# whxhcj/multimodal-S2UT

Hardware: AMD Instinct MI355X
Metric: audio-frames/sec/node, mm_s2ut_transformer fp16, max-tokens 40000, 1/2/4/8 GPUs (higher is better)
Workload: dtype fp16; 1 GPU; mm_s2ut_transformer base (ViT-768 image feats, multimodal_attention+gate); model=mm_s2ut_transformer, parallelism=dp1, front_end=GPU fbank+CMVN in step

## Files before the change

### multimodal-s2ut_amd/csrc/gemm.hip

```cpp
#include <stdlib.h>

#include <algorithm>
#include <mutex>

#include "gemm_common.h"

namespace {

#include "gemm_skinny.h"

template <bool KC>
MMS_DEV void load_tile(const h16* __restrict__ X, long ld, int rows_total, int kdim,
                       int row0, int k0, int kend, s16x8 (&r)[4]) {
  const int t = threadIdx.x;
#pragma unroll
  for (int i = 0; i < 4; ++i) {
    const int id = t + i * NT;
    s16x8 v = {0, 0, 0, 0, 0, 0, 0, 0};
    if (KC) {
      const int row = id >> 3, c = id & 7;
      const int gr = row0 + row, gk = k0 + c * 8;
      if (gr < rows_total) {
        const h16* src = X + (long)gr * ld + gk;
        if (gk + 8 <= kend) {
          v = *reinterpret_cast<const s16x8*>(src);
        } else {
#pragma unroll
          for (int e = 0; e < 8; ++e)
            if (gk + e < kend) v[e] = reinterpret_cast<const short*>(src)[e];
        }
      }
    } else {
      const int kr = id >> 4, c = id & 15;
      const int gk = k0 + kr, gr = row0 + c * 8;
      if (gk < kend) {
        const h16* src = X + (long)gk * ld + gr;
        if (gr + 8 <= rows_total) {
          v = *reinterpret_cast<const s16x8*>(src);
        } else {
#pragma unroll
          for (int e = 0; e < 8; ++e)
            if (gr + e < rows_total) v[e] = reinterpret_cast<const short*>(src)[e];
        }
      }
    }
    r[i] = v;
  }
  (void)kdim;
}

template <bool KC>
MMS_DEV void store_tile(char* lds, const s16x8 (&r)[4]) {
  const int t = threadIdx.x;
#pragma unroll
  for (int i = 0; i < 4; ++i) {
    const int id = t + i * NT;
    int off;
    if (KC) {
      const int row = id >> 3, c = id & 7;
      off = row * 128 + ((c ^ (row & 7)) << 4);
    } else {
      const int kr = id >> 4, c = id & 15;
      off = kr * 256 + ((c ^ swz_mn(kr)) << 4);
    }
    *reinterpret_cast<s16x8*>(lds + off) = r[i];
  }
}

template <bool A_KC, bool B_KC, int EPI>
__global__ void __launch_bounds__(NT, 2) gemm_kernel(GemmP P, int tiles_m, int tiles_n, int total) {
  const unsigned long long t_start = P.stamps ? stamp_now() : 0ull;
  if (P.thresh) P.seed = mms_step_seed(P.seed);
  __shared__ __attribute__((aligned(16))) char smem[4 * TILE_BYTES];
  int z, tm, tn;
  tile_coords(blockIdx.x, tiles_m, tiles_n, total, z, tm, tn, P.group_m);
  const int zb = z / P.splitk, zs = z % P.splitk;
  const int z1 = zb / P.bdiv, z2 = zb % P.bdiv;
  const h16* A = P.A + z1 * P.sA1 + z2 * P.sA2;
  const h16* B = P.B + z1 * P.sB1 + z2 * P.sB2;
  const int kbeg = zs * P.kchunk;
  const int kend = min(P.K, kbeg + P.kchunk);
  const int bm = tm * BM, bn = tn * BN;
  const int lane = threadIdx.x & 63, wid = threadIdx.x >> 6;
  const int wm = wid >> 1, wn = wid & 1;

#define SA(s) (smem + (2 * (s)) * TILE_BYTES)
#define SB(s) (smem + (2 * (s) + 1) * TILE_BYTES)

  f32x4 acc[4][4];
#pragma unroll
  for (int i = 0; i < 4; ++i)
#pragma unroll
    for (int j = 0; j < 4; ++j) acc[i][j] = f32x4{0.f, 0.f, 0.f, 0.f};

  s16x8 ra[4], rb[4];
  const int nk = (kend - kbeg + BK - 1) / BK;
  if (nk > 0) {
    load_tile<A_KC>(A, P.lda, P.M, P.K, bm, kbeg, kend, ra);
    load_tile<B_KC>(B, P.ldb, P.N, P.K, bn, kbeg, kend, rb);
    store_tile<A_KC>(SA(0), ra);
    store_tile<B_KC>(SB(0), rb);
  }
  __syncthreads();
  for (int kt = 0; kt < nk; ++kt) {
    const int cur = kt & 1;
    const bool more = kt + 1 < nk;
    if (more) {
      const int k0 = kbeg + (kt + 1) * BK;
      load_tile<A_KC>(A, P.lda, P.M, P.K, bm, k0, kend, ra);
      load_tile<B_KC>(B, P.ldb, P.N, P.K, bn, k0, kend, rb);
    }
#pragma unroll
    for (int kk = 0; kk < 2; ++kk) {
      h16x8 fa[4], fb[4];
#pragma unroll
      for (int i = 0; i < 4; ++i) fa[i] = read_frag<A_KC>(SA(cur), wm * 64 + i * 16, kk, lane);
#pragma unroll
      for (int j = 0; j < 4; ++j) fb[j] = read_frag<B_KC>(SB(cur), wn * 64 + j * 16, kk, lane);
#pragma unroll
      for (int i = 0; i < 4; ++i)
#pragma unroll
        for (int j = 0; j < 4; ++j)
          acc[i][j] = __builtin_amdgcn_mfma_f32_16x16x32_f16(fb[j], fa[i], acc[i][j], 0, 0, 0);
    }
    if (more) {
      store_tile<A_KC>(SA(cur ^ 1), ra);
      store_tile<B_KC>(SB(cur ^ 1), rb);
    }
    __syncthreads();
  }
#undef SA
#undef SB

  char* Cz;
  if (EPI == MMS_EPI_F32)
    Cz = reinterpret_cast<char*>(P.C) + (z1 * P.sC1 + z2 * P.sC2 + zs * P.sCsplit) * 4;
  else
    Cz = reinterpret_cast<char*>(P.C) + (z1 * P.sC1 + z2 * P.sC2) * 2;
  const h16* auxz = P.aux ? P.aux + z1 * P.sX1 + z2 * P.sX2 : nullptr;
  staged_epilogue<EPI>(P, smem, acc, bm, bn, wm, wn, wid, lane, Cz, auxz);
  stamp_end(P.stamps, t_start);
}




template <bool A_KC, bool B_KC, int EPI, int STAGES, bool RS, bool PRI>
MMS_DEV void dma_gemm_tile(const GemmP& P, char* smem, int z, int tm, int tn) {
  const int zb = z / P.splitk, zs = z % P.splitk;
  const int z1 = zb / P.bdiv, z2 = zb % P.bdiv;
  const int kbeg = zs * P.kchunk;
  const int kend = min(P.K, kbeg + P.kchunk);
  const int bm = tm * BM, bn = tn * BN;
  const int lane = threadIdx.x & 63;
  const int wid = __builtin_amdgcn_readfirstlane(threadIdx.x >> 6);
  const int wm = wid >> 1, wn = wid & 1;
  const h16* Ab = P.A + z1 * P.sA1 + z2 * P.sA2 + (A_KC ? 0 : (long)kbeg * P.lda);
  const h16* Bb = P.B + z1 * P.sB1 + z2 * P.sB2 + (B_KC ? 0 : (long)kbeg * P.ldb);
  const long a_ext = A_KC ? ((long)(P.M - 1) * P.lda + P.K) * 2
                          : ((long)(kend - kbeg - 1) * P.lda + ((P.M + 7) & ~7)) * 2;
  const long b_ext = B_KC ? ((long)(P.N - 1) * P.ldb + P.K) * 2
                          : ((long)(kend - kbeg - 1) * P.ldb + ((P.N + 7) & ~7)) * 2;
  const __amdgpu_buffer_rsrc_t ra = __builtin_amdgcn_make_buffer_rsrc((void*)Ab, (short)0, (int)a_ext, 0x00020000);
  const __amdgpu_buffer_rsrc_t rb = __builtin_amdgcn_make_buffer_rsrc((void*)Bb, (short)0, (int)b_ext, 0x00020000);
#define SA(s) (smem + (2 * (s)) * TILE_BYTES)
#define SB(s) (smem + (2 * (s) + 1) * TILE_BYTES)
  f32x4 acc[4][4];
#pragma unroll
  for (int i = 0; i < 4; ++i)
#pragma unroll
    for (int j = 0; j < 4; ++j) acc[i][j] = f32x4{0.f, 0.f, 0.f, 0.f};

  f32x4 rs[4];
  const bool do_rs = RS && tn == 0 && wn == 0 && (P.rowsum || P.rowsum16);
  if (RS) {
#pragma unroll
    for (int i = 0; i < 4; ++i) rs[i] = f32x4{0.f, 0.f, 0.f, 0.f};
  }
  h16x8 ones;
#pragma unroll
  for (int e = 0; e < 8; ++e) ones[e] = (h16)1.f;
  const int nk = (kend - kbeg + BK - 1) / BK;
  auto k_rel = [&](int t, bool kc) { return kc ? kbeg + t * BK : t * BK; };
#pragma unroll
  for (int s = 0; s < STAGES - 1; ++s) {
    if (s < nk) {
      dma_tile<A_KC>(ra, SA(s), P.lda, bm, k_rel(s, A_KC), wid, lane);
      dma_tile<B_KC>(rb, SB(s), P.ldb, bn, k_rel(s, B_KC), wid, lane);
    }
  }
#ifndef MMS_GEMM_DMA_AFTER_READS
#define MMS_GEMM_DMA_AFTER_READS 0
#endif
  constexpr bool READ_FIRST = !A_KC || !B_KC || MMS_GEMM_DMA_AFTER_READS;
  for (int kt = 0; kt < nk; ++kt) {
    const int younger = min(STAGES - 2, nk - 1 - kt);
    if (STAGES >= 3 && younger >= 1) wait_vm<8>(); else wait_vm<0>();
    __builtin_amdgcn_s_barrier();
    const int nxt = kt + STAGES - 1;
    const int cur = kt % STAGES;
    if (!READ_FIRST && nxt < nk) {
      const int sb = nxt % STAGES;
      dma_tile<A_KC>(ra, SA(sb), P.lda, bm, k_rel(nxt, A_KC), wid, lane);
      dma_tile<B_KC>(rb, SB(sb), P.ldb, bn, k_rel(nxt, B_KC), wid, lane);
    }
    h16x8 fa2[2][4], fb2[2][4];
    {
#pragma unroll
      for (int kk = 0; kk < 2; ++kk) {
#pragma unroll
        for (int i = 0; i < 4; ++i) fa2[kk][i] = read_frag<A_KC>(SA(cur), wm * 64 + i * 16, kk, lane);
#pragma unroll
        for (int j = 0; j < 4; ++j) fb2[kk][j] = read_frag<B_KC>(SB(cur), wn * 64 + j * 16, kk, lane);
      }
    }
    if (READ_FIRST && nxt < nk) {
      const int sb = nxt % STAGES;
      dma_tile<A_KC>(ra, SA(sb), P.lda, bm, k_rel(nxt, A_KC), wid, lane);
      dma_tile<B_KC>(rb, SB(sb), P.ldb, bn, k_rel(nxt, B_KC), wid, lane);
    }
#pragma unroll
    for (int kk = 0; kk < 2; ++kk) {
      h16x8 fa[4], fb[4];
#pragma unroll
      for (int i = 0; i < 4; ++i) { fa[i] = fa2[kk][i]; fb[i] = fb2[kk][i]; }
      if (PRI) __builtin_amdgcn_s_setprio(1);
#pragma unroll
      for (int i = 0; i < 4; ++i)
#pragma unroll
        for (int j = 0; j < 4; ++j)
          acc[i][j] = __builtin_amdgcn_mfma_f32_16x16x32_f16(fb[j], fa[i], acc[i][j], 0, 0, 0);
      if (PRI) __builtin_amdgcn_s_setprio(0);
      if (RS && do_rs) {
#pragma unroll
        for (int i = 0; i < 4; ++i) rs[i] = __builtin_amdgcn_mfma_f32_16x16x32_f16(ones, fa[i], rs[i], 0, 0, 0);
      }
    }
  }
#undef SA
#undef SB
  if (RS && do_rs && lane < 16) {
#pragma unroll
    for (int i = 0; i < 4; ++i) {
      const int m = bm + wm * 64 + i * 16 + lane;
      if (m < P.M) {
        if (P.rowsum16) P.rowsum16[m] = (h16)(rs[i][0] * P.alpha);
        else P.rowsum[(long)zs * P.ld_rowsum + m] = rs[i][0] * P.alpha;
      }
    }
  }
  char* Cz;
  if (EPI == MMS_EPI_F32)
    Cz = reinterpret_cast<char*>(P.C) + (z1 * P.sC1 + z2 * P.sC2 + zs * P.sCsplit) * 4;
  else
    Cz = reinterpret_cast<char*>(P.C) + (z1 * P.sC1 + z2 * P.sC2) * 2;
  const h16* auxz = P.aux ? P.aux + z1 * P.sX1 + z2 * P.sX2 : nullptr;
  __syncthreads();
#ifdef MMS_GEMM_NOEPI
#pragma unroll
  for (int i = 0; i < 4; ++i)
#pragma unroll
    for (int j = 0; j < 4; ++j) asm volatile("" :: "v"(acc[i][j]));
  (void)Cz; (void)auxz;
#else
  staged_epilogue<EPI>(P, smem, acc, bm, bn, wm, wn, wid, lane, Cz, auxz);
#endif
}

template <bool A_KC, bool B_KC, int EPI, int STAGES, bool RS = false>
__global__ void __launch_bounds__(NT, (STAGES <= 2 ? 2 : 1)) gemm_dma_kernel(GemmP P, int tiles_m, int tiles_n, int total) {
  const unsigned long long t_start = P.stamps ? stamp_now() : 0ull;
  if (P.thresh) P.seed = mms_step_seed(P.seed);
  __shared__ __attribute__((aligned(16))) char smem[STAGES * 2 * TILE_BYTES];
  int z, tm, tn;
  tile_coords(blockIdx.x, tiles_m, tiles_n, total, z, tm, tn, P.group_m);
  dma_gemm_tile<A_KC, B_KC, EPI, STAGES, RS, PRIO && EPI != MMS_EPI_F32>(P, smem, z, tm, tn);
  stamp_end(P.stamps, t_start);
}

template <int EPI, int FRT>
__global__ void __launch_bounds__(NT, 2) gemm_tall_kernel(GemmP P, int tiles_m, int tiles_n, int total) {
  constexpr int BMT = 32 * FRT, TILE_T = BMT * 64 * 2;
  constexpr int SMEM = 2 * (TILE_T + TILE_BYTES) > 4 * 64 * 64 * 4 ? 2 * (TILE_T + TILE_BYTES) : 4 * 64 * 64 * 4;
  const unsigned long long t_start = P.stamps ? stamp_now() : 0ull;
  if (P.thresh) P.seed = mms_step_seed(P.seed);
  __shared__ __attribute__((aligned(16))) char smem[SMEM];
  int z, tm, tn;
  tile_coords(blockIdx.x, tiles_m, tiles_n, total, z, tm, tn, P.group_m);
  (void)z;
  const int bm = tm * BMT, bn = tn * BN;
  const int lane = threadIdx.x & 63;
  const int wid = __builtin_amdgcn_readfirstlane(threadIdx.x >> 6);
  const int wm = wid >> 1, wn = wid & 1;
  const long a_ext = ((long)(P.M - 1) * P.lda + P.K) * 2;
  const long b_ext = ((long)(P.N - 1) * P.ldb + P.K) * 2;
  const __amdgpu_buffer_rsrc_t ra = __builtin_amdgcn_make_buffer_rsrc((void*)P.A, (short)0, (int)a_ext, 0x00020000);
  const __amdgpu_buffer_rsrc_t rb = __builtin_amdgcn_make_buffer_rsrc((void*)P.B, (short)0, (int)b_ext, 0x00020000);
#define SA(s) (smem + (s) * (TILE_T + TILE_BYTES))
#define SB(s) (SA(s) + TILE_T)
  auto dma_a = [&](char* lds, int k0) {
#ifndef MMS_GEMM_NODMA
#pragma unroll
    for (int x = 0; x < FRT; ++x) {
      const int ins = wid * FRT + x;
      const int row = ins * 8 + (lane >> 3), c = (lane & 7) ^ (row & 7);
      const int voff = (int)(((long)(bm + row) * P.lda + k0 + c * 8) * 2);
      __builtin_amdgcn_raw_ptr_buffer_load_lds(ra, (lds_void*)(lds + ins * 1024), 16, voff, 0, 0, 0);
    }
#endif
  };
  f32x4 acc[FRT][4];
#pragma unroll
  for (int i = 0; i < FRT; ++i)
#pragma unroll
    for (int j = 0; j < 4; ++j) acc[i][j] = f32x4{0.f, 0.f, 0.f, 0.f};
  const int nk = P.K / BK;
  if (nk > 0) {
    dma_a(SA(0), 0);
    dma_tile<true>(rb, SB(0), P.ldb, bn, 0, wid, lane);
  }
  constexpr bool PR = PRIO && EPI != MMS_EPI_F32;
  for (int kt = 0; kt < nk; ++kt) {
    wait_vm<0>();
    __builtin_amdgcn_s_barrier();
    const int cur = kt & 1;
    if (kt + 1 < nk) {
      dma_a(SA(cur ^ 1), (kt + 1) * BK);
      dma_tile<true>(rb, SB(cur ^ 1), P.ldb, bn, (kt + 1) * BK, wid, lane);
    }
    h16x8 fa2[2][FRT], fb2[2][4];
#pragma unroll
    for (int kk = 0; kk < 2; ++kk) {
#pragma unroll
      for (int i = 0; i < FRT; ++i) fa2[kk][i] = read_frag<true>(SA(cur), wm * 16 * FRT + i * 16, kk, lane);
#pragma unroll
      for (int j = 0; j < 4; ++j) fb2[kk][j] = read_frag<true>(SB(cur), wn * 64 + j * 16, kk, lane);
    }
#pragma unroll
    for (int kk = 0; kk < 2; ++kk) {
      if (PR) __builtin_amdgcn_s_setprio(1);
#pragma unroll
      for (int i = 0; i < FRT; ++i)
#pragma unroll
        for (int j = 0; j < 4; ++j)
          acc[i][j] = __builtin_amdgcn_mfma_f32_16x16x32_f16(fb2[kk][j], fa2[kk][i], acc[i][j], 0, 0, 0);
      if (PR) __builtin_amdgcn_s_setprio(0);
    }
  }
#undef SA
#undef SB
  __syncthreads();
  constexpr int WR = 16 * FRT, F1 = FRT < 4 ? FRT : 4;
  if constexpr (epi_regs<EPI>() && MMS_GEMM_REG_TALL) {
    if (reg_epilogue_ok(P)) {
      reg_epilogue<EPI, FRT, FRT * 2048>(P, smem, acc, bm + (WR - 64) * wm, bn, wm, wn, wid, lane, P.C);
      stamp_end(P.stamps, t_start);
      return;
    }
  }
  staged_epilogue<EPI, F1>(P, smem, reinterpret_cast<const f32x4(&)[F1][4]>(acc[0]), bm + (WR - 64) * wm, bn, wm,
                           wn, wid, lane, P.C, P.aux);
  if constexpr (FRT > 4) {
    __syncthreads();
    staged_epilogue<EPI, FRT - 4>(P, smem, reinterpret_cast<const f32x4(&)[FRT - 4][4]>(acc[4]),
                                  bm + (WR - 64) * wm + 64, bn, wm, wn, wid, lane, P.C, P.aux);
  }
  stamp_end(P.stamps, t_start);
}

constexpr int kGroupMax = 8;
struct GemmGroup {
  GemmP p[kGroupMax];
  int first[kGroupMax + 1];
  int tiles_m[kGroupMax], tiles_n[kGroupMax];
  int n;
  unsigned long long* stamps;
};

__global__ void __launch_bounds__(NT, 2) gemm_group_wgrad_kernel(GemmGroup G, int total) {
  const unsigned long long t_start = G.stamps ? stamp_now() : 0ull;
  __shared__ __attribute__((aligned(16))) char smem[2 * 2 * TILE_BYTES];
  const int q = total / 8, r = total % 8;
  for (int lin = blockIdx.x; lin < total; lin += gridDim.x) {
    if (lin != (int)blockIdx.x) __syncthreads();
    const int x = lin % 8;
    const int id = (x < r ? x * (q + 1) : r * (q + 1) + (x - r) * q) + lin / 8;
    int g = 0;
    while (g + 1 < G.n && id >= G.first[g + 1]) ++g;
    const GemmP& P = G.p[g];
    const int t = id - G.first[g], tiles_n = G.tiles_n[g];
    const int per_group = P.group_m * tiles_n;
    const int grp = t / per_group, first_m = grp * P.group_m;
    const int gsize = min(G.tiles_m[g] - first_m, P.group_m);
    const int w = t % per_group;
    dma_gemm_tile<false, false, MMS_EPI_F16, 2, true, false>(P, smem, 0, first_m + w % gsize, w / gsize);
  }
  stamp_end(G.stamps, t_start);
}

constexpr int BM2 = 256, BN2 = 256, NT2 = 512, SLOT2 = 2 * 2 * T32_BYTES;
constexpr int RING2 = 4;

template <bool KC>
MMS_DEV void dma_slot2(__amdgpu_buffer_rsrc_t rs, char* img, long ld, int row0, int k0rel, int wid, int lane) {
#pragma unroll
  for (int i = 0; i < 2; ++i) {
    const int ins = wid + 8 * i;
    const int half = ins >> 3, hi = ins & 7;
    const int r0 = row0 + half * 128;
    int voff;
    if (KC) {
      const int row = hi * 16 + (lane >> 2), slot = lane & 3;
      const int c = slot ^ swz32(row);
      voff = (int)(((long)(r0 + row) * ld + k0rel + c * 8) * 2);
    } else {
      const int kr = hi * 4 + (lane >> 4), slot = lane & 15;
      const int c = slot ^ swz_mn(kr);
      voff = (int)(((long)(k0rel + kr) * ld + r0 + c * 8) * 2);
    }
    __builtin_amdgcn_raw_ptr_buffer_load_lds(rs, (lds_void*)(img + half * T32_BYTES + hi * 1024), 16, voff, 0, 0, 0);
  }
}

template <bool A_KC, bool B_KC, int EPI, int RING>
__global__ void __launch_bounds__(NT2, 2) gemm256p_kernel(GemmP P, int tiles_m, int tiles_n, int total) {
  const unsigned long long t_start = P.stamps ? stamp_now() : 0ull;
  if (P.thresh) P.seed = mms_step_seed(P.seed);
  __shared__ __attribute__((aligned(16))) char smem[RING * SLOT2];
  int z, tm, tn;
  tile_coords(blockIdx.x, tiles_m, tiles_n, total, z, tm, tn, P.group_m);
  const int zb = z / P.splitk, zs = z % P.splitk;
  const int z1 = zb / P.bdiv, z2 = zb % P.bdiv;
  const int kbeg = zs * P.kchunk;
  const int kend = min(P.K, kbeg + P.kchunk);
  const int bm = tm * BM2, bn = tn * BN2;
  const int lane = threadIdx.x & 63;
  const int wid = __builtin_amdgcn_readfirstlane(threadIdx.x >> 6);
  const int wr = wid >> 2, wc = wid & 3;
  const h16* Ab = P.A + z1 * P.sA1 + z2 * P.sA2 + (A_KC ? 0 : (long)kbeg * P.lda);
  const h16* Bb = P.B + z1 * P.sB1 + z2 * P.sB2 + (B_KC ? 0 : (long)kbeg * P.ldb);
  const long a_ext = A_KC ? ((long)(P.M - 1) * P.lda + P.K) * 2
                          : ((long)(kend - kbeg - 1) * P.lda + ((P.M + 7) & ~7)) * 2;
  const long b_ext = B_KC ? ((long)(P.N - 1) * P.ldb + P.K) * 2
                          : ((long)(kend - kbeg - 1) * P.ldb + ((P.N + 7) & ~7)) * 2;
  const __amdgpu_buffer_rsrc_t ra = __builtin_amdgcn_make_buffer_rsrc((void*)Ab, (short)0, (int)a_ext, 0x00020000);
  const __amdgpu_buffer_rsrc_t rb = __builtin_amdgcn_make_buffer_rsrc((void*)Bb, (short)0, (int)b_ext, 0x00020000);
#define SLA(s) (smem + (s) * SLOT2)
#define SLB(s) (smem + (s) * SLOT2 + 2 * T32_BYTES)
  f32x4 acc[8][4];
#pragma unroll
  for (int i = 0; i < 8; ++i)
#pragma unroll
    for (int j = 0; j < 4; ++j) acc[i][j] = f32x4{0.f, 0.f, 0.f, 0.f};
  const int nk = (kend - kbeg + BK32 - 1) / BK32;
  auto k_rel = [&](int t, bool kc) { return kc ? kbeg + t * BK32 : t * BK32; };
#pragma unroll
  for (int t = 0; t < RING - 1; ++t) {
    if (t < nk) {
      dma_slot2<A_KC>(ra, SLA(t), P.lda, bm, k_rel(t, A_KC), wid, lane);
      dma_slot2<B_KC>(rb, SLB(t), P.ldb, bn, k_rel(t, B_KC), wid, lane);
    }
  }
  const int a_half = wr * T32_BYTES, b_half = (wc >> 1) * T32_BYTES, b_sub = (wc & 1) * 64;
  auto wait_slot = [&](int want, int issued) {
    const int younger = min(issued, nk - 1) - want;
    if (RING >= 5 && younger >= 3) wait_vm<12>();
    else if (younger >= 2) wait_vm<8>();
    else if (younger == 1) wait_vm<4>();
    else wait_vm<0>();
  };
  h16x8 faA[4], fbA[4], faB[4], fbB[4];
  if (nk > 0) {
    wait_slot(0, RING - 2);
    __builtin_amdgcn_s_barrier();
#pragma unroll
    for (int j = 0; j < 4; ++j) fbA[j] = read_frag32<B_KC>(SLB(0) + b_half, b_sub + j * 16, lane);
#pragma unroll
    for (int i = 0; i < 4; ++i) faA[i] = read_frag32<A_KC>(SLA(0) + a_half, i * 16, lane);
  }
  auto slot = [&](int ks, const h16x8 (&fa_lo)[4], const h16x8 (&fb)[4], h16x8 (&fan)[4], h16x8 (&fbn)[4]) {
    const int cur = ks % RING;
    h16x8 fa_hi[4];
#pragma unroll
    for (int i = 0; i < 4; ++i) fa_hi[i] = read_frag32<A_KC>(SLA(cur) + a_half, 64 + i * 16, lane);
    __builtin_amdgcn_s_setprio(1);
#pragma unroll
    for (int i = 0; i < 4; ++i)
#pragma unroll
      for (int j = 0; j < 4; ++j)
        acc[i][j] = __builtin_amdgcn_mfma_f32_16x16x32_f16(fb[j], fa_lo[i], acc[i][j], 0, 0, 0);
    __builtin_amdgcn_s_setprio(0);
    wait_slot(ks + 1, ks + RING - 2);
    __builtin_amdgcn_s_barrier();
    const int nxt = ks + RING - 1;
    if (nxt < nk) {
      const int sn = nxt % RING;
      dma_slot2<A_KC>(ra, SLA(sn), P.lda, bm, k_rel(nxt, A_KC), wid, lane);
      dma_slot2<B_KC>(rb, SLB(sn), P.ldb, bn, k_rel(nxt, B_KC), wid, lane);
    }
    const int c1 = (ks + 1) % RING;
#pragma unroll
    for (int j = 0; j < 4; ++j) fbn[j] = read_frag32<B_KC>(SLB(c1) + b_half, b_sub + j * 16, lane);
#pragma unroll
    for (int i = 0; i < 4; ++i) fan[i] = read_frag32<A_KC>(SLA(c1) + a_half, i * 16, lane);
    __builtin_amdgcn_s_setprio(1);
// ... 741 lines not shown
```

### multimodal-s2ut_amd/csrc/gemm_common.h

```cpp
#pragma once
#include "common.h"
#include "../../include/mms2ut.h"

namespace mmsg {
struct GemmP {
  const h16* A; const h16* B; void* C;
  int M, N, K;
  long lda, ldb, ldc;
  int bdiv;
  long sA1, sA2, sB1, sB2, sC1, sC2;
  int splitk; int kchunk; long sCsplit;
  float alpha;
  const h16* bias;
  const h16* aux; long ldaux; long sX1, sX2;
  h16* out2; long ldo2;
  float p; uint32_t thresh; uint64_t seed, offset; long ld_rng;
  int vec16;
  float* rowsum; long ld_rowsum;
  h16* rowsum16;
  int group_m;
  unsigned long long* stamps;
};

}
// ... 221 lines not shown
    h16x8 gv;
#pragma unroll
    for (int r = 0; r < 8; ++r) gv[r] = (h16)g[r];
    *reinterpret_cast<h16x8*>(P.out2 + (long)m * P.ldo2 + n) = gv;
  } else if (EPI == MMS_EPI_RELU_DROP_BWD) {
    float h[8];
    ld8(auxz + (long)m * P.ldaux + n, h);
#pragma unroll
    for (int r = 0; r < 8; ++r) o[r] = h[r] > 0.f ? x[r] * dscale : 0.f;
  } else if (EPI == MMS_EPI_F16_ACC) {
    float c[8];
    ld8(C + n, c);
#pragma unroll
    for (int r = 0; r < 8; ++r) o[r] = c[r] + x[r];
  } else if (EPI == MMS_EPI_GELU_DROP) {
    h16x8 zv;
#pragma unroll
    for (int r = 0; r < 8; ++r) {
      zv[r] = (h16)x[r];
      o[r] = keep[r] ? gelu_((float)zv[r]) * dscale : 0.f;
    }
    *reinterpret_cast<h16x8*>(P.out2 + (long)m * P.ldo2 + n) = zv;
  } else if (EPI == MMS_EPI_GELU_DROP_BWD) {
    float z[8];
    ld8(auxz + (long)m * P.ldaux + n, z);
#pragma unroll
    for (int r = 0; r < 8; ++r) o[r] = keep[r] ? x[r] * dscale * gelu_grad_(z[r]) : 0.f;
  } else {
#pragma unroll
    for (int r = 0; r < 8; ++r) o[r] = x[r];
  }
  h16x8 ov8;
#pragma unroll
  for (int r = 0; r < 8; ++r) ov8[r] = (h16)o[r];
  *reinterpret_cast<h16x8*>(C + n) = ov8;
}

MMS_DEV void tile_coords(int bid, int tiles_m, int tiles_n, int total, int& z, int& tm, int& tn, int GROUP_M) {
  const int q = total / 8, r = total % 8, x = bid % 8;
  const int id = (x < r ? x * (q + 1) : r * (q + 1) + (x - r) * q) + bid / 8;
  const int ntiles = tiles_m * tiles_n;
  z = id / ntiles;
  const int t = id % ntiles;
  const int per_group = GROUP_M * tiles_n;
  const int g = t / per_group, first_m = g * GROUP_M;
  const int gsize = min(tiles_m - first_m, GROUP_M);
  const int w = t % per_group;
  tm = first_m + w % gsize;
  tn = w / gsize;
}

template <int EPI>
constexpr bool epi_drops() {
  return EPI == MMS_EPI_RELU_DROP || EPI == MMS_EPI_DROP_RESID || EPI == MMS_EPI_GELU_DROP ||
         EPI == MMS_EPI_GELU_DROP_BWD;
}

#ifndef MMS_GEMM_REG_EPI
#define MMS_GEMM_REG_EPI 1
#endif
#ifndef MMS_GEMM_REG_STAGED
#define MMS_GEMM_REG_STAGED 1
#endif
#ifndef MMS_GEMM_REG_TALL
#define MMS_GEMM_REG_TALL 1
#endif
template <int EPI>
constexpr bool epi_regs() {
  return MMS_GEMM_REG_EPI && (EPI == MMS_EPI_F16 || EPI == MMS_EPI_RELU_DROP);
}

MMS_DEV bool reg_epilogue_ok(const GemmP& P) { return P.vec16 == 1 && P.N % 64 == 0; }

template <int EPI, int FR, int SLOTB>
MMS_DEV void reg_epilogue(const GemmP& P, char* smem, const f32x4 (&acc)[FR][4], int bm, int bn, int wm, int wn,
                          int wid, int lane, void* Cz) {
  static_assert(SLOTB >= FR * 2048, "staging slot too small");
  if (bn + wn * 64 >= P.N) return;
  char* stage = smem + wid * SLOTB;
  const int rl = lane & 15, g = lane >> 4;
  const int m0 = bm + wm * 64 + rl, nw = bn + wn * 64 + 4 * g;
  float bv[4][4];
#pragma unroll
  for (int j = 0; j < 4; ++j)
#pragma unroll
    for (int e = 0; e < 4; ++e) bv[j][e] = 0.f;
  if (P.bias) {
#pragma unroll
    for (int j = 0; j < 4; ++j) {
      const h16x4 b4 = *reinterpret_cast<const h16x4*>(P.bias + nw + 16 * j);
#pragma unroll
      for (int e = 0; e < 4; ++e) bv[j][e] = (float)b4[e];
    }
  }
  constexpr bool DROPS = EPI == MMS_EPI_RELU_DROP;
  const float dscale = P.thresh ? 1.f / (1.f - P.p) : 1.f;
  uint32_t hmix = 0, pbase = 0;
  bool fast = false;
  if (DROPS && P.thresh) {
    const uint64_t cf = P.offset + (uint64_t)m0 * P.ld_rng + nw;
    const uint64_t cl = P.offset + (uint64_t)(m0 + 16 * (FR - 1)) * P.ld_rng + nw + 51;
    const bool sh = mms_same_hi(cf, cl) && ((cf & 1) == 0) && ((P.ld_rng & 1) == 0);
    hmix = mms_hi_mix(P.seed, cf);
    pbase = (uint32_t)(cf >> 1);
    fast = __all(sh);
  }
#pragma unroll
  for (int i = 0; i < FR; ++i) {
    const int rr = i * 16 + rl;
#pragma unroll
    for (int j = 0; j < 4; ++j) {
      float x[4];
#pragma unroll
      for (int e = 0; e < 4; ++e) x[e] = acc[i][j][e] * P.alpha + bv[j][e];
      bool keep[4] = {true, true, true, true};
      if (DROPS && P.thresh && fast) {
        const uint32_t p0 = pbase + (uint32_t)(8 * i) * (uint32_t)P.ld_rng + 8 * j;
        const uint32_t h0 = mms_mix32(p0 ^ hmix), h1 = mms_mix32((p0 + 1) ^ hmix);
        keep[0] = (h0 & 0xffffU) >= P.thresh;
        keep[1] = (h0 >> 16) >= P.thresh;
        keep[2] = (h1 & 0xffffU) >= P.thresh;
        keep[3] = (h1 >> 16) >= P.thresh;
      } else if (DROPS && P.thresh) {
        mms_keep4(P.seed, P.offset + (uint64_t)(m0 + 16 * i) * P.ld_rng + nw + 16 * j, P.thresh, keep);
      }
      h16x4 o4;
#pragma unroll
      for (int e = 0; e < 4; ++e) {
        float o;
        if (EPI == MMS_EPI_RELU_DROP) o = keep[e] ? fmaxf(x[e], 0.f) * dscale : 0.f;
        else o = x[e];
        o4[e] = (h16)o;
      }
      const int ch = (2 * j + (g >> 1)) ^ ((rr >> 1) & 7);
      *reinterpret_cast<h16x4*>(stage + rr * 128 + (ch << 4) + (((g ^ rr) & 1) << 3)) = o4;
    }
  }
  asm volatile("s_waitcnt lgkmcnt(0)" ::: "memory");
  __builtin_amdgcn_wave_barrier();
  const int q = lane & 7;
  h16* C = reinterpret_cast<h16*>(Cz);
  const int n = bn + wn * 64 + 8 * q;
#pragma unroll
  for (int pass = 0; pass < 2 * FR; ++pass) {
    const int rr = pass * 8 + (lane >> 3);
    typedef unsigned int u32x4_ __attribute__((ext_vector_type(4)));
    u32x4_ v = *reinterpret_cast<const u32x4_*>(stage + rr * 128 + ((q ^ ((rr >> 1) & 7)) << 4));
    if (rr & 1) v = u32x4_{v[2], v[3], v[0], v[1]};
    const int m = bm + wm * 64 + rr;
    if (m < P.M) *reinterpret_cast<u32x4_*>(C + (long)m * P.ldc + n) = v;
  }
}

template <int EPI, int FR = 4, int SLOT = 64 * 64>
MMS_DEV void staged_epilogue(const GemmP& P, char* smem, const f32x4 (&acc)[FR][4], int bm, int bn,
                             int wm, int wn, int wid, int lane, void* Cz, const h16* auxz) {
  static_assert(SLOT >= FR * 16 * 64, "staging slot too small");
  if constexpr (epi_regs<EPI>() && MMS_GEMM_REG_STAGED) {
    if (reg_epilogue_ok(P)) {
      reg_epilogue<EPI, FR, SLOT * 4>(P, smem, acc, bm, bn, wm, wn, wid, lane, Cz);
      return;
    }
  }
  constexpr int PASSES = FR * 2;
  float* stage = reinterpret_cast<float*>(smem) + wid * SLOT;
#pragma unroll
  for (int i = 0; i < FR; ++i)
#pragma unroll
    for (int j = 0; j < 4; ++j) {
      const int r = i * 16 + (lane & 15);
      const int c = j * 4 + (lane >> 4);
      *reinterpret_cast<f32x4*>(stage + r * 64 + ((c ^ (r & 15)) << 2)) = acc[i][j];
    }
  __syncthreads();
  const int q = lane & 7;
  const int n = bn + wn * 64 + 8 * q;
  auto stage8 = [&](int r, float (&v)[8]) {
    const f32x4 lo = *reinterpret_cast<const f32x4*>(stage + r * 64 + (((2 * q) ^ (r & 15)) << 2));
    const f32x4 hi = *reinterpret_cast<const f32x4*>(stage + r * 64 + (((2 * q + 1) ^ (r & 15)) << 2));
    v[0] = lo[0]; v[1] = lo[1]; v[2] = lo[2]; v[3] = lo[3];
    v[4] = hi[0]; v[5] = hi[1]; v[6] = hi[2]; v[7] = hi[3];
  };
  constexpr bool LOADS = EPI == MMS_EPI_DROP_RESID || EPI == MMS_EPI_GATE || EPI == MMS_EPI_RELU_DROP_BWD ||
                         EPI == MMS_EPI_F16_ACC || EPI == MMS_EPI_GELU_DROP_BWD;
  if (EPI == MMS_EPI_F32 || !(P.vec16 && n + 7 < P.N)) {
#pragma unroll 2
    for (int pass = 0; pass < PASSES; ++pass) {
      const int r = pass * 8 + (lane >> 3);
      float v[8];
      stage8(r, v);
      epilogue_store8<EPI>(P, Cz, auxz, bm + wm * 64 + r, n, v);
    }
    return;
  }
  const int m0 = bm + wm * 64 + (lane >> 3);
  float bv[8] = {0.f, 0.f, 0.f, 0.f, 0.f, 0.f, 0.f, 0.f};
  if (EPI != MMS_EPI_RELU_DROP_BWD && EPI != MMS_EPI_GELU_DROP_BWD && P.bias) {
    const h16x8 b8 = *reinterpret_cast<const h16x8*>(P.bias + n);
#pragma unroll
    for (int e = 0; e < 8; ++e) bv[e] = (float)b8[e];
  }
  h16* C = reinterpret_cast<h16*>(Cz);
  h16x8 ax[8], ax2[8];
  const h16x8 z8 = {(h16)0.f, (h16)0.f, (h16)0.f, (h16)0.f, (h16)0.f, (h16)0.f, (h16)0.f, (h16)0.f};
#pragma unroll
  for (int pass = 0; pass < PASSES; ++pass) {
    const int m = m0 + 8 * pass;
    ax[pass] = z8;
    ax2[pass] = z8;
    if (LOADS && m < P.M) {
      if (EPI == MMS_EPI_F16_ACC) {
        ax[pass] = *reinterpret_cast<const h16x8*>(C + (long)m * P.ldc + n);
      } else {
        ax[pass] = *reinterpret_cast<const h16x8*>(auxz + (long)m * P.ldaux + n);
        if (EPI == MMS_EPI_GATE) ax2[pass] = *reinterpret_cast<const h16x8*>(auxz + (long)m * P.ldaux + P.N + n);
      }
    }
  }
  const float dscale = P.thresh ? 1.f / (1.f - P.p) : 1.f;
  constexpr bool DROPS = EPI == MMS_EPI_RELU_DROP || EPI == MMS_EPI_DROP_RESID || EPI == MMS_EPI_GELU_DROP ||
                         EPI == MMS_EPI_GELU_DROP_BWD;
  uint32_t hmix = 0, pbase = 0;
  bool same_hi = false, fast = false;
  if (DROPS && P.thresh) {
    const uint64_t cf = P.offset + (uint64_t)m0 * P.ld_rng + n;
    const uint64_t cl = P.offset + (uint64_t)(m0 + 8 * (PASSES - 1)) * P.ld_rng + n + 7;
    same_hi = mms_same_hi(cf, cl) && ((cf & 1) == 0) && ((P.ld_rng & 1) == 0);
    hmix = mms_hi_mix(P.seed, cf);
    pbase = (uint32_t)(cf >> 1);
    fast = __all(same_hi);
  }
#pragma unroll
  for (int pass = 0; pass < PASSES; ++pass) {
    const int m = m0 + 8 * pass;
    if (m >= P.M) continue;
    float x[8];
    stage8(pass * 8 + (lane >> 3), x);
#pragma unroll
    for (int e = 0; e < 8; ++e) x[e] = x[e] * P.alpha + bv[e];
    bool keep[8] = {true, true, true, true, true, true, true, true};
    if (DROPS && P.thresh && fast) {
      const uint32_t p0 = pbase + (uint32_t)(4 * pass) * (uint32_t)P.ld_rng;
#pragma unroll
      for (int h = 0; h < 4; ++h) {
        const uint32_t hv = mms_mix32((p0 + h) ^ hmix);
        keep[2 * h] = (hv & 0xffffU) >= P.thresh;
        keep[2 * h + 1] = (hv >> 16) >= P.thresh;
      }
    } else if (DROPS && P.thresh) {
      const uint64_t c0 = P.offset + (uint64_t)m * P.ld_rng + n;
      bool k0[4], k1[4];
      if (same_hi) {
        mms_keep4_hi(hmix, c0, P.thresh, k0);
        mms_keep4_hi(hmix, c0 + 4, P.thresh, k1);
      } else {
        mms_keep4(P.seed, c0, P.thresh, k0);
        mms_keep4(P.seed, c0 + 4, P.thresh, k1);
      }
#pragma unroll
      for (int e = 0; e < 4; ++e) { keep[e] = k0[e]; keep[e + 4] = k1[e]; }
    }
    h16x8 o8;
    if (EPI == MMS_EPI_GATE) {
      h16x8 g8;
#pragma unroll
      for (int e = 0; e < 8; ++e) {
        const float g = sigmoidf_(x[e]), ov = (float)ax[pass][e], tv = (float)ax2[pass][e];
        g8[e] = (h16)g;
        o8[e] = (h16)(tv + g * (ov - tv));
      }
      *reinterpret_cast<h16x8*>(P.out2 + (long)m * P.ldo2 + n) = g8;
    } else if (EPI == MMS_EPI_GELU_DROP) {
      h16x8 z8;
#pragma unroll
      for (int e = 0; e < 8; ++e) {
        z8[e] = (h16)x[e];
        o8[e] = (h16)(keep[e] ? gelu_((float)z8[e]) * dscale : 0.f);
      }
      *reinterpret_cast<h16x8*>(P.out2 + (long)m * P.ldo2 + n) = z8;
    } else if (EPI == MMS_EPI_GELU_DROP_BWD) {
#pragma unroll
      for (int e = 0; e < 8; ++e)
        o8[e] = (h16)(keep[e] ? x[e] * dscale * gelu_grad_((float)ax[pass][e]) : 0.f);
    } else {
#pragma unroll
      for (int e = 0; e < 8; ++e) {
        float o;
        if (EPI == MMS_EPI_RELU_DROP) o = keep[e] ? fmaxf(x[e], 0.f) * dscale : 0.f;
        else if (EPI == MMS_EPI_DROP_RESID) o = (float)ax[pass][e] + (keep[e] ? x[e] * dscale : 0.f);
        else if (EPI == MMS_EPI_RELU_DROP_BWD) o = (float)ax[pass][e] > 0.f ? x[e] * dscale : 0.f;
        else if (EPI == MMS_EPI_F16_ACC) o = (float)ax[pass][e] + x[e];
        else o = x[e];
        o8[e] = (h16)o;
      }
    }
#if defined(MMS_LAB_NOSTORE)
    asm volatile("" ::"v"(o8));
#elif defined(MMS_GEMM_NT_STORE)
    __builtin_nontemporal_store(o8, reinterpret_cast<h16x8*>(C + (long)m * P.ldc + n));
#else
    *reinterpret_cast<h16x8*>(C + (long)m * P.ldc + n) = o8;
#endif
  }
}

constexpr int BK32 = 32, T32_BYTES = 128 * 32 * 2, ST32 = 4;
MMS_DEV int swz32(int r) { return ((r >> 1) & 1) | (((r >> 2) & 1) << 1); }

template <bool KC>
MMS_DEV h16x8 read_frag32(const char* lds, int sub, int lane) {
  if (KC) {
    const int r = sub + (lane & 15);
    const int c = lane >> 4;
    s16x8 v = *reinterpret_cast<const s16x8*>(lds + r * 64 + ((c ^ swz32(r)) << 4));
    return __builtin_bit_cast(h16x8, v);
  }
  return read_frag<false>(lds, sub, 0, lane);
}

typedef __attribute__((address_space(3))) void lds_void;

template <bool KC>
MMS_DEV void dma_tile(__amdgpu_buffer_rsrc_t rs, char* lds, long ld, int row0, int k0rel, int wid, int lane) {
#ifdef MMS_GEMM_NODMA
  return;
#endif
#pragma unroll
  for (int i = 0; i < 4; ++i) {
    const int ins = wid * 4 + i;
    int voff;
    if (KC) {
      const int row = ins * 8 + (lane >> 3), slot = lane & 7;
      const int c = slot ^ (row & 7);
      voff = (int)(((long)(row0 + row) * ld + k0rel + c * 8) * 2);
    } else {
      const int kr = ins * 4 + (lane >> 4), slot = lane & 15;
      const int c = slot ^ swz_mn(kr);
      voff = (int)(((long)(k0rel + kr) * ld + row0 + c * 8) * 2);
    }
    __builtin_amdgcn_raw_ptr_buffer_load_lds(rs, (lds_void*)(lds + ins * 1024), 16, voff, 0, 0, 0);
  }
}

template <int N>
MMS_DEV void wait_vm() {
  asm volatile("s_waitcnt vmcnt(%0)" ::"n"(N) : "memory");
}

#define MMS_EPI_CASES CASE(MMS_EPI_F16) CASE(MMS_EPI_RELU_DROP) CASE(MMS_EPI_DROP_RESID) CASE(MMS_EPI_F32) \
    CASE(MMS_EPI_GATE) CASE(MMS_EPI_RELU_DROP_BWD) CASE(MMS_EPI_F16_ACC) CASE(MMS_EPI_GELU_DROP) CASE(MMS_EPI_GELU_DROP_BWD)

}
```

Baseline: 2.021 million audio-frames/s.

## Permute B-tile rows so GEMM epilogue writes contiguous fp16 vectors and prefetches operands

The B-operand DMA now loads rows in a permuted order (perm_row). Each lane's accumulator columns then line up as contiguous 8-element fp16 groups, so a new perm_epilogue can apply bias, dropout, residual or gate and pack 16-byte vectors without the fp32 LDS staging shuffle. Epilogue operands (bias, residual or aux, gate inputs) are prefetched during the last K iteration so their latency overlaps the final MFMAs. This costs extra registers for the prefetched operands and more code paths, and the permuted-row mapping must stay consistent with the fragment layout.

```diff
diff --git a/multimodal-s2ut_amd/csrc/gemm.hip b/multimodal-s2ut_amd/csrc/gemm.hip
--- a/multimodal-s2ut_amd/csrc/gemm.hip
+++ b/multimodal-s2ut_amd/csrc/gemm.hip
@@ -2,6 +2,7 @@
 
 #include <algorithm>
 #include <mutex>
+#include <type_traits>
 
 #include "gemm_common.h"
 
@@ -182,27 +183,40 @@
   for (int e = 0; e < 8; ++e) ones[e] = (h16)1.f;
   const int nk = (kend - kbeg + BK - 1) / BK;
   auto k_rel = [&](int t, bool kc) { return kc ? kbeg + t * BK : t * BK; };
+  constexpr bool PERM_T = A_KC && B_KC && !RS && epi_perm<EPI>();
+  const bool perm = PERM_T && reg_epilogue_ok(P);
+  char* Cz;
+  if (EPI == MMS_EPI_F32)
+    Cz = reinterpret_cast<char*>(P.C) + (z1 * P.sC1 + z2 * P.sC2 + zs * P.sCsplit) * 4;
+  else
+    Cz = reinterpret_cast<char*>(P.C) + (z1 * P.sC1 + z2 * P.sC2) * 2;
+  const h16* auxz = P.aux ? P.aux + z1 * P.sX1 + z2 * P.sX2 : nullptr;
+  PermOperands<EPI, 4> op;
 #pragma unroll
   for (int s = 0; s < STAGES - 1; ++s) {
     if (s < nk) {
       dma_tile<A_KC>(ra, SA(s), P.lda, bm, k_rel(s, A_KC), wid, lane);
-      dma_tile<B_KC>(rb, SB(s), P.ldb, bn, k_rel(s, B_KC), wid, lane);
+      dma_tile<B_KC>(rb, SB(s), P.ldb, bn, k_rel(s, B_KC), wid, lane, perm);
     }
   }
 #ifndef MMS_GEMM_DMA_AFTER_READS
 #define MMS_GEMM_DMA_AFTER_READS 0
 #endif
   constexpr bool READ_FIRST = !A_KC || !B_KC || MMS_GEMM_DMA_AFTER_READS;
-  for (int kt = 0; kt < nk; ++kt) {
+  auto k_step = [&](int kt, auto last_tag) {
+    constexpr bool LAST = decltype(last_tag)::value;
     const int younger = min(STAGES - 2, nk - 1 - kt);
     if (STAGES >= 3 && younger >= 1) wait_vm<8>(); else wait_vm<0>();
     __builtin_amdgcn_s_barrier();
     const int nxt = kt + STAGES - 1;
     const int cur = kt % STAGES;
+    if constexpr (PERM_T && LAST) {
+      if (perm) perm_prefetch<EPI, 4>(P, op, bm, bn, wm, wn, lane, Cz, auxz);
+    }
     if (!READ_FIRST && nxt < nk) {
       const int sb = nxt % STAGES;
       dma_tile<A_KC>(ra, SA(sb), P.lda, bm, k_rel(nxt, A_KC), wid, lane);
-      dma_tile<B_KC>(rb, SB(sb), P.ldb, bn, k_rel(nxt, B_KC), wid, lane);
+      dma_tile<B_KC>(rb, SB(sb), P.ldb, bn, k_rel(nxt, B_KC), wid, lane, perm);
     }
     h16x8 fa2[2][4], fb2[2][4];
     {
@@ -217,7 +231,7 @@
     if (READ_FIRST && nxt < nk) {
       const int sb = nxt % STAGES;
       dma_tile<A_KC>(ra, SA(sb), P.lda, bm, k_rel(nxt, A_KC), wid, lane);
-      dma_tile<B_KC>(rb, SB(sb), P.ldb, bn, k_rel(nxt, B_KC), wid, lane);
+      dma_tile<B_KC>(rb, SB(sb), P.ldb, bn, k_rel(nxt, B_KC), wid, lane, perm);
     }
 #pragma unroll
     for (int kk = 0; kk < 2; ++kk) {
@@ -236,6 +250,13 @@
         for (int i = 0; i < 4; ++i) rs[i] = __builtin_amdgcn_mfma_f32_16x16x32_f16(ones, fa[i], rs[i], 0, 0, 0);
       }
     }
+  };
+  if constexpr (PERM_T) {
+    for (int kt = 0; kt < nk - 1; ++kt) k_step(kt, std::false_type{});
+    if (nk > 0) k_step(nk - 1, std::true_type{});
+    else if (perm) perm_prefetch<EPI, 4>(P, op, bm, bn, wm, wn, lane, Cz, auxz);
+  } else {
+    for (int kt = 0; kt < nk; ++kt) k_step(kt, std::false_type{});
   }
 #undef SA
 #undef SB
@@ -249,12 +270,9 @@
       }
     }
   }
-  char* Cz;
-  if (EPI == MMS_EPI_F32)
-    Cz = reinterpret_cast<char*>(P.C) + (z1 * P.sC1 + z2 * P.sC2 + zs * P.sCsplit) * 4;
-  else
-    Cz = reinterpret_cast<char*>(P.C) + (z1 * P.sC1 + z2 * P.sC2) * 2;
-  const h16* auxz = P.aux ? P.aux + z1 * P.sX1 + z2 * P.sX2 : nullptr;
+#if MMS_GEMM_PERM_DIRECT
+  if (!perm)
+#endif
   __syncthreads();
 #ifdef MMS_GEMM_NOEPI
 #pragma unroll
@@ -263,6 +281,12 @@
     for (int j = 0; j < 4; ++j) asm volatile("" :: "v"(acc[i][j]));
   (void)Cz; (void)auxz;
 #else
+  if constexpr (PERM_T) {
+    if (perm) {
+      perm_epilogue<EPI, 4, 64 * 64 * 4>(P, smem, acc, op, bm, bn, wm, wn, wid, lane, Cz, auxz);
+      return;
+    }
+  }
   staged_epilogue<EPI>(P, smem, acc, bm, bn, wm, wn, wid, lane, Cz, auxz);
 #endif
 }
@@ -315,18 +339,26 @@
 #pragma unroll
     for (int j = 0; j < 4; ++j) acc[i][j] = f32x4{0.f, 0.f, 0.f, 0.f};
   const int nk = P.K / BK;
+  constexpr bool PERM_T = epi_perm<EPI>() && MMS_GEMM_REG_TALL;
+  const bool perm = PERM_T && reg_epilogue_ok(P);
+  constexpr int WR = 16 * FRT, F1 = FRT < 4 ? FRT : 4;
+  PermOperands<EPI, FRT> op;
   if (nk > 0) {
     dma_a(SA(0), 0);
-    dma_tile<true>(rb, SB(0), P.ldb, bn, 0, wid, lane);
+    dma_tile<true>(rb, SB(0), P.ldb, bn, 0, wid, lane, perm);
   }
   constexpr bool PR = PRIO && EPI != MMS_EPI_F32;
-  for (int kt = 0; kt < nk; ++kt) {
+  auto k_step = [&](int kt, auto last_tag) {
+    constexpr bool LAST = decltype(last_tag)::value;
     wait_vm<0>();
     __builtin_amdgcn_s_barrier();
     const int cur = kt & 1;
+    if constexpr (PERM_T && LAST) {
+      if (perm) perm_prefetch<EPI, FRT>(P, op, bm + (WR - 64) * wm, bn, wm, wn, lane, P.C, P.aux);
+    }
     if (kt + 1 < nk) {
       dma_a(SA(cur ^ 1), (kt + 1) * BK);
-      dma_tile<true>(rb, SB(cur ^ 1), P.ldb, bn, (kt + 1) * BK, wid, lane);
+      dma_tile<true>(rb, SB(cur ^ 1), P.ldb, bn, (kt + 1) * BK, wid, lane, perm);
     }
     h16x8 fa2[2][FRT], fb2[2][4];
 #pragma unroll
@@ -346,11 +378,27 @@
           acc[i][j] = __builtin_amdgcn_mfma_f32_16x16x32_f16(fb2[kk][j], fa2[kk][i], acc[i][j], 0, 0, 0);
       if (PR) __builtin_amdgcn_s_setprio(0);
     }
+  };
+  if constexpr (PERM_T) {
+    for (int kt = 0; kt < nk - 1; ++kt) k_step(kt, std::false_type{});
+    if (nk > 0) k_step(nk - 1, std::true_type{});
+    else if (perm) perm_prefetch<EPI, FRT>(P, op, bm + (WR - 64) * wm, bn, wm, wn, lane, P.C, P.aux);
+  } else {
+    for (int kt = 0; kt < nk; ++kt) k_step(kt, std::false_type{});
   }
 #undef SA
 #undef SB
+#if MMS_GEMM_PERM_DIRECT
+  if (!perm)
+#endif
   __syncthreads();
-  constexpr int WR = 16 * FRT, F1 = FRT < 4 ? FRT : 4;
+  if constexpr (PERM_T) {
+    if (perm) {
+      perm_epilogue<EPI, FRT, FRT * 2048>(P, smem, acc, op, bm + (WR - 64) * wm, bn, wm, wn, wid, lane, P.C, P.aux);
+      stamp_end(P.stamps, t_start);
+      return;
+    }
+  }
   if constexpr (epi_regs<EPI>() && MMS_GEMM_REG_TALL) {
     if (reg_epilogue_ok(P)) {
       reg_epilogue<EPI, FRT, FRT * 2048>(P, smem, acc, bm + (WR - 64) * wm, bn, wm, wn, wid, lane, P.C);
diff --git a/multimodal-s2ut_amd/csrc/gemm_common.h b/multimodal-s2ut_amd/csrc/gemm_common.h
--- a/multimodal-s2ut_amd/csrc/gemm_common.h
+++ b/multimodal-s2ut_amd/csrc/gemm_common.h
@@ -397,6 +397,189 @@
   }
 }
 
+#ifndef MMS_GEMM_PERM
+#define MMS_GEMM_PERM 1
+#endif
+#ifndef MMS_GEMM_PERM_DIRECT
+#define MMS_GEMM_PERM_DIRECT 0
+#endif
+template <int EPI>
+constexpr bool epi_perm() {
+  return MMS_GEMM_REG_EPI && MMS_GEMM_PERM &&
+         (EPI == MMS_EPI_F16 || EPI == MMS_EPI_RELU_DROP || EPI == MMS_EPI_DROP_RESID || EPI == MMS_EPI_GATE ||
+          EPI == MMS_EPI_RELU_DROP_BWD || EPI == MMS_EPI_F16_ACC);
+}
+MMS_DEV int perm_row(int r) { return (r & ~0x1c) | ((r & 0x0c) << 1) | ((r & 0x10) >> 2); }
+
+template <int EPI, int FR>
+struct PermOperands {
+  h16x8 ax[FR][2];
+  h16x8 ax2[EPI == MMS_EPI_GATE ? FR : 1][2];
+  h16x8 bias[2];
+};
+
+template <int EPI, int FR>
+constexpr bool perm_gate_late() { return EPI == MMS_EPI_GATE && FR > 4; }
+
+template <int EPI, int FR>
+MMS_DEV void perm_prefetch(const GemmP& P, PermOperands<EPI, FR>& op, int bm, int bn, int wm, int wn, int lane,
+                           const void* Cz, const h16* auxz) {
+  h16x8 z8;
+#pragma unroll
+  for (int e = 0; e < 8; ++e) z8[e] = (h16)0.f;
+  constexpr bool LOADS = (EPI == MMS_EPI_DROP_RESID || EPI == MMS_EPI_GATE || EPI == MMS_EPI_RELU_DROP_BWD ||
+                          EPI == MMS_EPI_F16_ACC) && !perm_gate_late<EPI, FR>();
+  op.bias[0] = op.bias[1] = z8;
+#pragma unroll
+  for (int i = 0; i < FR; ++i) op.ax[i][0] = op.ax[i][1] = z8;
+#pragma unroll
+  for (int i = 0; i < (EPI == MMS_EPI_GATE ? FR : 1); ++i) op.ax2[i][0] = op.ax2[i][1] = z8;
+  if (bn + wn * 64 >= P.N) return;
+  const int m0 = bm + wm * 64 + (lane & 15), nw = bn + wn * 64 + 8 * (lane >> 4);
+  if (EPI != MMS_EPI_RELU_DROP_BWD && P.bias) {
+#pragma unroll
+    for (int h = 0; h < 2; ++h) op.bias[h] = *reinterpret_cast<const h16x8*>(P.bias + nw + 32 * h);
+  }
+  if (LOADS) {
+    const h16* src = EPI == MMS_EPI_F16_ACC ? reinterpret_cast<const h16*>(Cz) : auxz;
+    const long ld = EPI == MMS_EPI_F16_ACC ? P.ldc : P.ldaux;
+#pragma unroll
+    for (int i = 0; i < FR; ++i) {
+      const int m = m0 + 16 * i;
+      if (m < P.M) {
+#pragma unroll
+        for (int h = 0; h < 2; ++h) {
+          op.ax[i][h] = *reinterpret_cast<const h16x8*>(src + (long)m * ld + nw + 32 * h);
+          if (EPI == MMS_EPI_GATE)
+            op.ax2[EPI == MMS_EPI_GATE ? i : 0][h] = *reinterpret_cast<const h16x8*>(src + (long)m * ld + P.N + nw + 32 * h);
+        }
+      }
+    }
+  }
+}
+
+template <int EPI, int FR, int SLOTB>
+MMS_DEV void perm_epilogue(const GemmP& P, char* smem, const f32x4 (&acc)[FR][4], PermOperands<EPI, FR>& op,
+                           int bm, int bn, int wm, int wn, int wid, int lane, void* Cz, const h16* auxz) {
+  static_assert(SLOTB >= FR * 2048, "staging slot too small");
+  if (bn + wn * 64 >= P.N) return;
+  constexpr bool GATE_LATE = perm_gate_late<EPI, FR>();
+  h16x8 nx[2], nx2[2];
+  auto load_gate = [&](int i) {
+    const int m = bm + wm * 64 + (lane & 15) + 16 * i;
+#pragma unroll
+    for (int h = 0; h < 2; ++h) {
+      nx[h] = nx2[h] = op.bias[h];
+      if (m < P.M) {
+        const h16* src = auxz + (long)m * P.ldaux + bn + wn * 64 + 8 * (lane >> 4) + 32 * h;
+        nx[h] = *reinterpret_cast<const h16x8*>(src);
+        nx2[h] = *reinterpret_cast<const h16x8*>(src + P.N);
+      }
+    }
+  };
+  if (GATE_LATE) load_gate(0);
+  char* stage = smem + wid * SLOTB;
+  const int rl = lane & 15, g = lane >> 4;
+  const int m0 = bm + wm * 64 + rl, nw = bn + wn * 64 + 8 * g;
+  h16* C = reinterpret_cast<h16*>(Cz);
+  float bv[2][8];
+#pragma unroll
+  for (int h = 0; h < 2; ++h)
+#pragma unroll
+    for (int e = 0; e < 8; ++e) bv[h][e] = (float)op.bias[h][e];
+  constexpr bool DROPS = EPI == MMS_EPI_RELU_DROP || EPI == MMS_EPI_DROP_RESID;
+  const float dscale = P.thresh ? 1.f / (1.f - P.p) : 1.f;
+  uint32_t hmix = 0, pbase = 0;
+  bool same_hi = false, fast = false;
+  if (DROPS && P.thresh) {
+    const uint64_t cf = P.offset + (uint64_t)m0 * P.ld_rng + nw;
+    const uint64_t cl = P.offset + (uint64_t)(m0 + 16 * (FR - 1)) * P.ld_rng + nw + 39;
+    same_hi = mms_same_hi(cf, cl) && ((cf & 1) == 0) && ((P.ld_rng & 1) == 0);
+    hmix = mms_hi_mix(P.seed, cf);
+    pbase = (uint32_t)(cf >> 1);
+    fast = __all(same_hi);
+  }
+#pragma unroll
+  for (int i = 0; i < FR; ++i) {
+    const int rr = i * 16 + rl, m = m0 + 16 * i;
+    if (GATE_LATE) {
+#pragma unroll
+      for (int h = 0; h < 2; ++h) { op.ax[0][h] = nx[h]; op.ax2[0][h] = nx2[h]; }
+      if (i + 1 < FR) load_gate(i + 1);
+    }
+#pragma unroll
+    for (int h = 0; h < 2; ++h) {
+      float x[8];
+#pragma unroll
+      for (int e = 0; e < 8; ++e) x[e] = acc[i][2 * h + (e >> 2)][e & 3] * P.alpha + bv[h][e];
+      bool keep[8] = {true, true, true, true, true, true, true, true};
+      if (DROPS && P.thresh && fast) {
+        const uint32_t p0 = pbase + (uint32_t)(8 * i) * (uint32_t)P.ld_rng + 16 * h;
+#pragma unroll
+        for (int t = 0; t < 4; ++t) {
+          const uint32_t hv = mms_mix32((p0 + t) ^ hmix);
+          keep[2 * t] = (hv & 0xffffU) >= P.thresh;
+          keep[2 * t + 1] = (hv >> 16) >= P.thresh;
+        }
+      } else if (DROPS && P.thresh) {
+        const uint64_t c0 = P.offset + (uint64_t)m * P.ld_rng + nw + 32 * h;
+        bool k0[4], k1[4];
+        if (same_hi) {
+          mms_keep4_hi(hmix, c0, P.thresh, k0);
+          mms_keep4_hi(hmix, c0 + 4, P.thresh, k1);
+        } else {
+          mms_keep4(P.seed, c0, P.thresh, k0);
+          mms_keep4(P.seed, c0 + 4, P.thresh, k1);
+        }
+#pragma unroll
+        for (int e = 0; e < 4; ++e) { keep[e] = k0[e]; keep[e + 4] = k1[e]; }
+      }
+      h16x8 o8;
+      if (EPI == MMS_EPI_GATE) {
+        h16x8 g8;
+#pragma unroll
+        for (int e = 0; e < 8; ++e) {
+          const float gt = sigmoidf_(x[e]), ov = (float)op.ax[GATE_LATE ? 0 : i][h][e];
+          const float tv = (float)op.ax2[(EPI == MMS_EPI_GATE && !GATE_LATE) ? i : 0][h][e];
+          g8[e] = (h16)gt;
+          o8[e] = (h16)(tv + gt * (ov - tv));
+        }
+        if (m < P.M) *reinterpret_cast<h16x8*>(P.out2 + (long)m * P.ldo2 + nw + 32 * h) = g8;
+      } else {
+#pragma unroll
+        for (int e = 0; e < 8; ++e) {
+          float o;
+          if (EPI == MMS_EPI_RELU_DROP) o = keep[e] ? fmaxf(x[e], 0.f) * dscale : 0.f;
+          else if (EPI == MMS_EPI_DROP_RESID) o = (float)op.ax[i][h][e] + (keep[e] ? x[e] * dscale : 0.f);
+          else if (EPI == MMS_EPI_RELU_DROP_BWD) o = (float)op.ax[i][h][e] > 0.f ? x[e] * dscale : 0.f;
+          else if (EPI == MMS_EPI_F16_ACC) o = (float)op.ax[i][h][e] + x[e];
+          else o = x[e];
+          o8[e] = (h16)o;
+        }
+      }
+#if MMS_GEMM_PERM_DIRECT
+      if (m < P.M) *reinterpret_cast<h16x8*>(C + (long)m * P.ldc + nw + 32 * h) = o8;
+#else
+      *reinterpret_cast<h16x8*>(stage + rr * 128 + (((4 * h + g) ^ (rr & 7)) << 4)) = o8;
+#endif
+    }
+  }
+#if !MMS_GEMM_PERM_DIRECT
+  asm volatile("s_waitcnt lgkmcnt(0)" ::: "memory");
+  __builtin_amdgcn_wave_barrier();
+  const int q = lane & 7;
+  const int n = bn + wn * 64 + 8 * q;
+#pragma unroll
+  for (int pass = 0; pass < 2 * FR; ++pass) {
+    const int rr = pass * 8 + (lane >> 3);
+    typedef unsigned int u32x4_ __attribute__((ext_vector_type(4)));
+    const u32x4_ v = *reinterpret_cast<const u32x4_*>(stage + rr * 128 + ((q ^ (rr & 7)) << 4));
+    const int mr = bm + wm * 64 + rr;
+    if (mr < P.M) *reinterpret_cast<u32x4_*>(C + (long)mr * P.ldc + n) = v;
+  }
+#endif
+}
+
 template <int EPI, int FR = 4, int SLOT = 64 * 64>
 MMS_DEV void staged_epilogue(const GemmP& P, char* smem, const f32x4 (&acc)[FR][4], int bm, int bn,
                              int wm, int wn, int wid, int lane, void* Cz, const h16* auxz) {
@@ -566,7 +749,8 @@
 typedef __attribute__((address_space(3))) void lds_void;
 
 template <bool KC>
-MMS_DEV void dma_tile(__amdgpu_buffer_rsrc_t rs, char* lds, long ld, int row0, int k0rel, int wid, int lane) {
+MMS_DEV void dma_tile(__amdgpu_buffer_rsrc_t rs, char* lds, long ld, int row0, int k0rel, int wid, int lane,
+                      bool perm = false) {
 #ifdef MMS_GEMM_NODMA
   return;
 #endif
@@ -577,7 +761,7 @@
     if (KC) {
       const int row = ins * 8 + (lane >> 3), slot = lane & 7;
       const int c = slot ^ (row & 7);
-      voff = (int)(((long)(row0 + row) * ld + k0rel + c * 8) * 2);
+      voff = (int)(((long)(row0 + (perm ? perm_row(row) : row)) * ld + k0rel + c * 8) * 2);
     } else {
       const int kr = ins * 4 + (lane >> 4), slot = lane & 15;
       const int c = slot ^ swz_mn(kr);
```

New measurement: 2.066 million audio-frames/s, median of 6. 1.02x the previous value.
